# spiraldb/fastlanes

Measured on AMD Instinct MI355X. Metric: billion integers/sec decoded (u32 width-7) + achieved HBM GB/s vs peak, 1-8 GPU, higher is better.
Workload: dtype u32

## Files before the change

fastlanes_amd/csrc/fl_pair.hip:

```cpp
#include "../../include/fastlanes_amd.h"
#include "../../include/fastlanes_amd_internal.h"
#include "fl_host.hpp"
#include "fl_stream.hpp"

#include <algorithm>
#include <atomic>
#include <cmath>
#include <memory>
#include <mutex>
#include <new>
#include <vector>

namespace {

using namespace fl;

int probe_classes(char* base, size_t n, size_t piece, int* classes, hipStream_t s)
{
    constexpr unsigned PROBE_WIDTH = 20;
    const size_t probe_blocks = std::min<size_t>(2000000, piece / (128 * PROBE_WIDTH));
    const size_t mask_off = piece - std::min<size_t>(piece / 2, (size_t)1 << 30);
    for (size_t g = 0; g < n; ++g) classes[g] = -1;
    if (n == 0 || probe_blocks == 0) return FL_OK;
    int rc = FL_OK;
    auto probe_ms = [&](size_t gi, size_t gm, float& ms) {
        const uint32_t* src = reinterpret_cast<const uint32_t*>(base + gi * piece);
        uint32_t* mask = reinterpret_cast<uint32_t*>(base + gm * piece + mask_off);
        return median_ms(s, 1, 3, [&] {
            const int saved = fl::window_override_this_thread();
            fl::window_override_this_thread() = fl::WINDOW_WHOLE;
            const int r = fl_u32_unpack_compare(PROBE_WIDTH, src, FL_CMP_LT, 1u << (PROBE_WIDTH - 1), probe_blocks, mask, s);
            fl::window_override_this_thread() = saved;
            return r;
        }, &ms);
    };
    float threshold = 0.f;
    std::vector<float> ms(n);
    for (int c = 0; c < 3 && rc == FL_OK; ++c) {
        size_t rep = 0;
        while (rep < n && classes[rep] != -1) ++rep;
        if (rep == n) break;
        classes[rep] = c;
        rc = fl_fill_random(base + rep * piece, probe_blocks * 128 * PROBE_WIDTH, 17 + rep, s);
        float slowest = 0.f, fastest = 1e30f;
        size_t others = 0;
        for (size_t g = 0; g < n && rc == FL_OK; ++g) {
            if (classes[g] != -1) continue;
            rc = probe_ms(rep, g, ms[g]);
            slowest = std::max(slowest, ms[g]);
            fastest = std::min(fastest, ms[g]);
            ++others;
        }
        if (rc != FL_OK || others == 0) break;
        if (threshold == 0.f) {
            if (slowest - fastest <= 0.05f * slowest) break;
            threshold = 0.5f * (slowest + fastest);
        }
        for (size_t g = 0; g < n; ++g)
            if (classes[g] == -1 && ms[g] > threshold) classes[g] = c;
    }
    return rc;
}

constexpr size_t PAIR_ALIGN = 256, PAIR_ZONE = (size_t)64 << 30, PAIR_MIB = (size_t)1 << 20, PAIR_GIB = (size_t)1 << 30;
constexpr size_t PAIR_INTERLEAVED_MIN = 8 * PAIR_GIB;
inline size_t pair_pad(size_t b) { return (b + PAIR_ALIGN - 1) & ~(PAIR_ALIGN - 1); }


std::mutex g_live_mutex;
std::vector<std::pair<uintptr_t, uintptr_t>> g_live;
std::atomic<int> g_live_count{0};
void live_pair_add(const char* va, size_t bytes)
{
    const uintptr_t lo = reinterpret_cast<uintptr_t>(va);
    std::lock_guard<std::mutex> lock(g_live_mutex);
    g_live.emplace_back(lo, lo + bytes);
    g_live_count.store((int)g_live.size(), std::memory_order_relaxed);
}
void live_pair_remove(const char* va)
{
    const uintptr_t lo = reinterpret_cast<uintptr_t>(va);
    std::lock_guard<std::mutex> lock(g_live_mutex);
    g_live.erase(std::remove_if(g_live.begin(), g_live.end(), [&](const auto& r) { return r.first == lo; }), g_live.end());
    g_live_count.store((int)g_live.size(), std::memory_order_relaxed);
}

constexpr int CACHE_DEVICES = 16;
std::vector<hipMemGenericAllocationHandle_t> g_chunk_cache[CACHE_DEVICES];
size_t g_chunk_cache_limit = 0;
std::atomic_flag g_chunk_cache_lock = ATOMIC_FLAG_INIT;
void recycle_chunk(hipMemGenericAllocationHandle_t h, int dev)
{
    bool kept = false;
    if (dev >= 0 && dev < CACHE_DEVICES) {
        while (g_chunk_cache_lock.test_and_set(std::memory_order_acquire)) {}
        if (g_chunk_cache[dev].size() < g_chunk_cache_limit) { g_chunk_cache[dev].push_back(h); kept = true; }
        g_chunk_cache_lock.clear(std::memory_order_release);
    }
    if (!kept) (void)hipMemRelease(h);
}
bool cached_chunk(int dev, hipMemGenericAllocationHandle_t& h)
{
    bool got = false;
    if (dev >= 0 && dev < CACHE_DEVICES) {
        while (g_chunk_cache_lock.test_and_set(std::memory_order_acquire)) {}
        if (!g_chunk_cache[dev].empty()) { h = g_chunk_cache[dev].back(); g_chunk_cache[dev].pop_back(); got = true; }
        g_chunk_cache_lock.clear(std::memory_order_release);
    }
    return got;
}

struct ColumnPair {
    void* bufs[3] = {nullptr, nullptr, nullptr};
    void *in = nullptr, *aux = nullptr, *out = nullptr;
    std::vector<hipMemGenericAllocationHandle_t> chunks;
    char* va = nullptr;
    size_t va_bytes = 0, chunk_bytes = 0, n_mapped = 0;
    int dev = -1;
    char class_map[96] = {0};
    ColumnPair() = default;
    ColumnPair(const ColumnPair&) = delete;
    ColumnPair& operator=(const ColumnPair&) = delete;
    ~ColumnPair()
    {
        for (void* b : bufs)
            if (b) (void)hipFree(b);
        if (n_mapped) {
            int cur = -1;
            const bool switched = hipGetDevice(&cur) == hipSuccess && cur != dev && hipSetDevice(dev) == hipSuccess;
            (void)hipDeviceSynchronize();
            if (switched) (void)hipSetDevice(cur);
        }
        for (size_t i = 0; i < n_mapped; ++i) (void)hipMemUnmap(va + i * chunk_bytes, chunk_bytes);
        for (auto h : chunks) recycle_chunk(h, dev);
        if (va) { live_pair_remove(va); (void)hipMemAddressFree(va, va_bytes); }
    }
};

std::atomic<uintptr_t> g_va_next{(uintptr_t)0x100000000000ull};
constexpr uintptr_t VA_ARENA_END = (uintptr_t)0x700000000000ull;
std::atomic_flag g_va_lock = ATOMIC_FLAG_INIT;
std::vector<std::pair<uintptr_t, uintptr_t>> g_va_used;

hipError_t reserve_fresh_range(size_t bytes, char** out)
{
    std::vector<void*> rejected;
    hipError_t e = hipErrorOutOfMemory;
    *out = nullptr;
    for (int attempt = 0; attempt < 6 && !*out; ++attempt) {
        const uintptr_t span = ((bytes + PAIR_GIB - 1) & ~(PAIR_GIB - 1)) + PAIR_GIB;
        const uintptr_t hint = g_va_next.fetch_add(span, std::memory_order_relaxed);
        if (hint + span > VA_ARENA_END) { e = hipErrorOutOfMemory; break; }
        void* p = nullptr;
        e = hipMemAddressReserve(&p, bytes, 2 * PAIR_MIB, reinterpret_cast<void*>(hint), 0);
        if (e != hipSuccess) { (void)hipGetLastError(); continue; }
        const uintptr_t lo = reinterpret_cast<uintptr_t>(p), hi = lo + bytes;
        while (g_va_lock.test_and_set(std::memory_order_acquire)) {}
        bool used = false;
        for (const auto& r : g_va_used) used = used || (lo < r.second && r.first < hi);
        if (!used) g_va_used.emplace_back(lo, hi);
        g_va_lock.clear(std::memory_order_release);
        if (used) { rejected.push_back(p); e = hipErrorOutOfMemory; }
        else *out = static_cast<char*>(p);
    }
    for (void* p : rejected) (void)hipMemAddressFree(p, bytes);
    return *out ? hipSuccess : e;
}

void choose_chunks(const std::vector<int>& cls, size_t n_in, size_t n_out, int out_classes, std::vector<int>& order, size_t* kept_out = nullptr)
{
    if (kept_out) *kept_out = 0;
    const size_t n = cls.size();
    order.clear();
    if (out_classes != 2) out_classes = 3;
    std::vector<int> by[4];
    for (size_t g = 0; g < n; ++g) by[cls[g] < 0 || cls[g] > 2 ? 3 : cls[g]].push_back((int)g);
    if (n_out == 0 || n_in + n_out > n) {
        for (size_t g = 0; g < n_in + n_out && g < n; ++g) order.push_back((int)g);
        return;
    }
    constexpr int TS = 64;
    std::vector<unsigned> pos((size_t)TS * 8);
    for (int t = 0; t < TS; ++t)
        for (int x = 0; x < 8; ++x) {
            const double p = (x + (t + 0.5) / TS) * (double)n_out / 8.0;
            pos[(size_t)t * 8 + x] = (unsigned)std::min<double>((double)n_out - 1, p);
        }
    struct Plan { std::vector<int> label; double cost; size_t kept; };
    auto plan = [&](int c) {
        Plan P;
        size_t avail[4] = {by[0].size(), by[1].size(), by[2].size(), by[3].size()};
        avail[c] -= n_in;
        static const double own_class_fee = [] { const char* e = getenv("FL_INTERNAL_OWN_CLASS_FEE"); return e ? atof(e) : 600.0; }();
        double fee[4] = {0, 0, 0, own_class_fee + 50.0};
        bool in_rotation[3], plentiful = true;
        for (int k = 0; k < 3; ++k) {
            in_rotation[k] = out_classes == 3 || k != c;
            if (in_rotation[k] && avail[k] * (size_t)out_classes < n_out + (size_t)out_classes - 1) plentiful = false;
        }
        for (int k = 0; k < 3; ++k) fee[k] = in_rotation[k] ? 0.0 : plentiful ? own_class_fee : 0.5 * own_class_fee;
        const int S[3] = {(c + 1) % 3, (c + 2) % 3, c};
        P.label.assign(n_out, 0);
        for (size_t j = 0; j < n_out; ++j) {
            const double at = (j + 0.5) * 8.0 / (double)n_out;
            const size_t x = (size_t)at, k = (size_t)((at - (double)x) * (double)n_out / 8.0);
            P.label[j] = S[(x + k) % (size_t)out_classes];
        }
        auto cost_of = [&](const std::vector<int>& lab) {
            double cost = 0.0;
            size_t used[4] = {0, 0, 0, 0};
            for (int k : lab) { ++used[k]; cost += fee[k] / (double)n_out; }
            for (int k = 0; k < 4; ++k) if (used[k] > avail[k]) cost += 10000.0 * (double)(used[k] - avail[k]);
            for (int t = 0; t < TS; ++t) {
                double cnt[4] = {0, 0, 0, 0};
                for (int x = 0; x < 8; ++x) cnt[lab[pos[(size_t)t * 8 + x]]] += 1.0;
                for (int k = 0; k < 4; ++k) cost += cnt[k] * cnt[k] * cnt[k] / TS;
            }
            return cost;
        };
        P.cost = cost_of(P.label);
        for (int sweep = 0; sweep < 12; ++sweep) {
            bool improved = false;
            for (size_t j = 0; j < n_out; ++j) {
                const int was = P.label[j];
                int best = was;
                for (int k = 0; k < 4; ++k) {
                    if (k == was) continue;
                    P.label[j] = k;
                    const double cst = cost_of(P.label);
                    if (cst < P.cost - 1e-9) { P.cost = cst; best = k; }
                }
                P.label[j] = best;
                improved = improved || best != was;
            }
            if (!improved) break;
        }
        size_t used[4] = {0, 0, 0, 0};
        for (int k : P.label) ++used[k];
        double off = 0.0;
        size_t outside = used[3];
        for (int k = 0; k < 3; ++k) {
            if (in_rotation[k]) off += std::max(0.0, std::fabs((double)used[k] - (double)n_out / out_classes) - 1.0);
            else outside += used[k];
        }
        const double kept = (double)n_out - (double)outside - off;
        P.kept = kept > 0.0 ? (size_t)kept : 0;
        for (int k = 0; k < 4; ++k) if (used[k] > avail[k]) P.kept = 0;
        return P;
    };
    int best_c = -1;
    Plan best;
    for (int c = 0; c < 3; ++c) {
        if (by[c].size() < n_in) continue;
        Plan P = plan(c);
        if (best_c < 0 || P.cost < best.cost - 1e-9 || (std::fabs(P.cost - best.cost) <= 1e-9 && by[c].size() > by[best_c].size())) { best = std::move(P); best_c = c; }
    }
    if (best_c < 0) {
        for (size_t g = 0; g < n_in + n_out && g < n; ++g) order.push_back((int)g);
        return;
    }
    if (kept_out) *kept_out = best.kept;
    size_t next[4] = {0, 0, 0, 0};
    for (size_t i = 0; i < n_in; ++i) order.push_back(by[best_c][next[best_c]++]);
    for (size_t j = 0; j < n_out; ++j) {
        int k = best.label[j];
        if (next[k] >= by[k].size()) {
            k = -1;
            for (int q = 0; q < 4; ++q) if (next[q] < by[q].size() && (k < 0 || by[q].size() - next[q] > by[k].size() - next[k])) k = q;
            if (k < 0) break;
        }
        order.push_back(by[k][next[k]++]);
    }
}
}

bool fl::fl_in_constructed_pair(std::initializer_list<const void*> ptrs)
{
    if (g_live_count.load(std::memory_order_relaxed) == 0) return false;
    std::lock_guard<std::mutex> lock(g_live_mutex);
    for (const auto& [lo, hi] : g_live) {
        int inside = 0;
        for (const void* p : ptrs) {
            const uintptr_t a = reinterpret_cast<uintptr_t>(p);
            inside += (a >= lo && a < hi);
        }
        if (inside >= 2) return true;
    }
    return false;
}

namespace {

std::mutex g_construct_mutex;

hipError_t pair_alloc_interleaved(size_t in_bytes, size_t aux_bytes, size_t out_bytes, hipStream_t s, ColumnPair& p, int& rc)
{
    std::lock_guard<std::mutex> one_at_a_time(g_construct_mutex);
    rc = FL_OK;
    int dev = 0, vmm = 0;
    hipError_t e = hipGetDevice(&dev);
    if (e == hipSuccess) e = hipDeviceGetAttribute(&vmm, hipDeviceAttributeVirtualMemoryManagementSupported, dev);
    if (e != hipSuccess) return e;
    if (!vmm) return hipErrorNotSupported;
    const size_t in_span = pair_pad(in_bytes) + pair_pad(aux_bytes), total = in_span + pair_pad(out_bytes);
    const size_t chunk = PAIR_GIB;
    const size_t n_in = std::max<size_t>(1, (in_span + chunk - 1) / chunk), n_out = std::max<size_t>(1, (pair_pad(out_bytes) + chunk - 1) / chunk);
    const int out_classes = pair_pad(out_bytes) >= 3 * in_span ? 2 : 3;
    size_t n_pool = std::max(std::max(std::max(3 * n_in + (out_classes == 3 ? n_out : 0), (3 * n_out + 1) / 2), 2 * (n_in + n_out)), 48 * PAIR_GIB / chunk);
    size_t free_b = 0, total_b = 0;
    if (hipMemGetInfo(&free_b, &total_b) == hipSuccess && free_b > 3 * PAIR_GIB) n_pool = std::min(n_pool, (free_b - 2 * PAIR_GIB) / chunk);
    if (n_pool < n_in + n_out) return hipErrorOutOfMemory;
    hipMemAllocationProp prop{};
    prop.type = hipMemAllocationTypePinned;
    prop.location.type = hipMemLocationTypeDevice;
    prop.location.id = dev;
    hipMemAccessDesc acc{};
    acc.location = prop.location;
    acc.flags = hipMemAccessFlagsProtReadWrite;
    std::vector<hipMemGenericAllocationHandle_t> pool;
    auto drop_pool = [&] { for (auto h : pool) recycle_chunk(h, dev); pool.clear(); };
    p.dev = dev;
    const size_t pool_cap = free_b > 3 * PAIR_GIB ? (free_b - 2 * PAIR_GIB) / chunk : n_pool;
    std::vector<int> cls, order;
    for (int round = 0;; ++round) {
        pool.reserve(n_pool);
        while (pool.size() < n_pool) {
            hipMemGenericAllocationHandle_t h;
            if (!cached_chunk(dev, h) && hipMemCreate(&h, chunk, &prop, 0) != hipSuccess) { (void)hipGetLastError(); break; }
            pool.push_back(h);
        }
        if (pool.size() < n_in + n_out) { drop_pool(); return hipErrorOutOfMemory; }
        cls.assign(pool.size(), -1);
        char* scratch = nullptr;
        e = reserve_fresh_range(pool.size() * chunk, &scratch);
        if (e != hipSuccess) { drop_pool(); return e; }
        size_t mapped = 0;
        for (; mapped < pool.size() && e == hipSuccess; ++mapped) e = hipMemMap(scratch + mapped * chunk, chunk, 0, pool[mapped], 0);
        if (e != hipSuccess) --mapped;
        if (e == hipSuccess) e = hipMemSetAccess(scratch, pool.size() * chunk, &acc, 1);
        if (e == hipSuccess) rc = probe_classes(scratch, pool.size(), chunk, cls.data(), s);
        if (e == hipSuccess && rc == FL_OK) e = hipStreamSynchronize(s);
        for (size_t i = 0; i < mapped; ++i) (void)hipMemUnmap(scratch + i * chunk, chunk);
        (void)hipMemAddressFree(scratch, pool.size() * chunk);
        if (e != hipSuccess || rc != FL_OK) { drop_pool(); return e; }
        size_t kept = 0;
        choose_chunks(cls, n_in, n_out, out_classes, order, &kept);
        const bool complete = order.size() == n_in + n_out;
        const size_t bigger = std::min(std::min(pool_cap, std::max<size_t>(3 * (n_in + n_out), 96)), pool.size() + std::max<size_t>(pool.size() / 2, 8));
        if ((complete && 10 * kept >= 9 * n_out) || round == 3 || pool.size() < n_pool || bigger <= pool.size()) {
            if (!complete) { drop_pool(); return hipErrorOutOfMemory; }
            break;
        }
        n_pool = bigger;
    }
    std::vector<char> keep(pool.size(), 0);
    for (int g : order) keep[g] = 1;
    p.chunk_bytes = chunk;
    p.va_bytes = order.size() * chunk;
    e = reserve_fresh_range(p.va_bytes, &p.va);
    for (size_t i = 0; i < order.size() && e == hipSuccess; ++i) {
        e = hipMemMap(p.va + i * chunk, chunk, 0, pool[order[i]], 0);
        if (e == hipSuccess) p.n_mapped = i + 1;
    }
    if (e == hipSuccess) e = hipMemSetAccess(p.va, p.va_bytes, &acc, 1);
    for (size_t g = 0; g < pool.size(); ++g) {
        if (keep[g]) p.chunks.push_back(pool[g]);
        else recycle_chunk(pool[g], dev);
    }
    pool.clear();
    if (e != hipSuccess) return e;
    for (size_t i = 0; i < order.size() && i + 1 < sizeof p.class_map; ++i) p.class_map[i] = cls[order[i]] < 0 ? '?' : (char)('A' + cls[order[i]]);
    p.in = p.va;
    p.aux = aux_bytes ? p.va + pair_pad(in_bytes) : nullptr;
    p.out = p.va + n_in * chunk;
    live_pair_add(p.va, p.va_bytes);
    return hipSuccess;
}

hipError_t pair_alloc(int layout, size_t in_bytes, size_t aux_bytes, size_t out_bytes, hipStream_t s, ColumnPair& p, int& rc)
{
    rc = FL_OK;
    if (layout == FL_LAYOUT_INTERLEAVED && pair_pad(in_bytes) + pair_pad(aux_bytes) + pair_pad(out_bytes) >= PAIR_INTERLEAVED_MIN)
        return pair_alloc_interleaved(in_bytes, aux_bytes, out_bytes, s, p, rc);
    if (layout == FL_LAYOUT_SEPARATE || layout == FL_LAYOUT_INTERLEAVED) {
        hipError_t e = hipMalloc(&p.bufs[0], in_bytes ? in_bytes : PAIR_ALIGN);
        if (e == hipSuccess && aux_bytes) e = hipMalloc(&p.bufs[1], aux_bytes);
        if (e == hipSuccess) e = hipMalloc(&p.bufs[2], out_bytes ? out_bytes : PAIR_ALIGN);
        if (e != hipSuccess) return e;
        p.in = p.bufs[0]; p.aux = p.bufs[1]; p.out = p.bufs[2];
        return hipSuccess;
    }
    const size_t in_end = pair_pad(in_bytes) + pair_pad(aux_bytes), half = pair_pad(out_bytes) / 2;
    size_t k = 1;
    while (k * PAIR_ZONE < half + in_end) {
        if (++k > 8) return hipErrorOutOfMemory;
    }
    const size_t out_off = (k * PAIR_ZONE - half) & ~(PAIR_ALIGN - 1);
    hipError_t e = hipMalloc(&p.bufs[0], out_off + pair_pad(out_bytes));
    if (e != hipSuccess) return e;
    char* base = static_cast<char*>(p.bufs[0]);
    p.in = base;
    p.aux = aux_bytes ? base + pair_pad(in_bytes) : nullptr;
    p.out = base + out_off;
    return hipSuccess;
}

int pair_probe(const ColumnPair& p, size_t in_bytes, size_t aux_bytes, size_t out_bytes, hipStream_t s, double& gbps)
{
    const size_t big = in_bytes > out_bytes ? in_bytes : out_bytes;
    const size_t n_units = big / 4096;
    gbps = 0.0;
    if (n_units < 1024) return FL_OK;
    auto unit = [&](size_t bytes) { size_t u = bytes / n_units & ~(size_t)15; return u > 4096 ? 4096 : u; };
    BareArgs a{static_cast<const char*>(p.in), static_cast<const char*>(p.aux), static_cast<char*>(p.out), n_units, 0,
               (unsigned)unit(in_bytes), aux_bytes >= n_units * 128 ? 128u : 0u, (unsigned)unit(out_bytes), 63u};
    if (a.out_unit == 0) return FL_OK;
    float ms = 0.f;
    const int rc = median_ms(s, 2, 5, [&] { return hip_status(launch_bare_stream(a, true, a.in_unit > a.out_unit ? 8 : 6, WINDOW_WHOLE, s)); }, &ms);
    if (rc != FL_OK) return rc;
    if (!(ms > 0.f)) return FL_OK;
    gbps = (double)n_units * (a.in_unit + a.aux_unit + a.out_unit) / (ms * 1e6);
    return FL_OK;
}

bool replaces_kept(int cand, double gbps, int kept, double best)
{
    return kept < 0 || gbps > best * (cand == FL_LAYOUT_ZONED ? 1.02 : 1.01);
}
constexpr int PROBE_ORDER[3] = {FL_LAYOUT_INTERLEAVED, FL_LAYOUT_SEPARATE, FL_LAYOUT_ZONED};
}

extern "C" {

int fl_internal_probe_memory_classes(void* slab, size_t slab_bytes, int* classes, void* stream)
{
    const size_t n_granules = slab_bytes / FL_INTERNAL_GRANULE_BYTES;
    if (n_granules == 0) return FL_OK;
    if (!slab || !classes) return FL_ERR_NULL;
    if (misaligned(slab)) return FL_ERR_ALIGN;
    return probe_classes(static_cast<char*>(slab), n_granules, FL_INTERNAL_GRANULE_BYTES, classes, static_cast<hipStream_t>(stream));
}

int fl_column_pair_alloc(size_t in_bytes, size_t aux_bytes, size_t out_bytes, int layout, void* stream, void** in, void** aux, void** out,
                         void** handle, int* layout_kept, uint32_t* probe_gbps)
{
    if (!in || !out || !handle || (aux_bytes && !aux)) return FL_ERR_NULL;
    if (layout < 0 || layout >= FL_LAYOUT_COUNT) return FL_ERR_INDEX;
    FL_DEVICE_TIER(stream);
    hipStream_t s = static_cast<hipStream_t>(stream);
    *in = *out = *handle = nullptr;
    if (aux) *aux = nullptr;
    if (probe_gbps) for (int i = 0; i < FL_LAYOUT_COUNT; ++i) probe_gbps[i] = 0;
    std::unique_ptr<ColumnPair> kept;
    int kept_layout = -1;
    const size_t biggest = in_bytes > out_bytes ? in_bytes : out_bytes;
    if (layout == FL_LAYOUT_PROBE && biggest / 4096 < 1024) layout = FL_LAYOUT_SEPARATE;
    if (layout != FL_LAYOUT_PROBE) {
        kept.reset(new (std::nothrow) ColumnPair);
        if (!kept) return hip_fail(hipErrorOutOfMemory);
        int rc = FL_OK;
        if (hipError_t e = pair_alloc(layout, in_bytes, aux_bytes, out_bytes, s, *kept, rc); e != hipSuccess || rc != FL_OK)
            return rc != FL_OK ? rc : hip_fail(e);
        kept_layout = layout;
    } else {
        double best = -1.0;
        const bool large = pair_pad(in_bytes) + pair_pad(aux_bytes) + pair_pad(out_bytes) >= PAIR_INTERLEAVED_MIN;
        for (int cand : PROBE_ORDER) {
            if (cand == FL_LAYOUT_INTERLEAVED && !large) continue;
            std::unique_ptr<ColumnPair> p(new (std::nothrow) ColumnPair);
            int prc = FL_OK;
            if (!p || pair_alloc(cand, in_bytes, aux_bytes, out_bytes, s, *p, prc) != hipSuccess || prc != FL_OK) { (void)hipGetLastError(); continue; }
            double gbps = 0.0;
            if (const int r = pair_probe(*p, in_bytes, aux_bytes, out_bytes, s, gbps); r != FL_OK) return r;
            if (probe_gbps) probe_gbps[cand] = (uint32_t)(gbps + 0.5);
            if (replaces_kept(cand, gbps, kept_layout, best)) { kept = std::move(p); best = gbps; kept_layout = cand; }
        }
        if (!kept) return hip_fail(hipErrorOutOfMemory);
    }
    *in = kept->in;
    if (aux) *aux = kept->aux;
    *out = kept->out;
    if (layout_kept) *layout_kept = kept_layout;
    *handle = kept.release();
    return FL_OK;
}

int fl_column_pair_free(void* handle)
{
    delete static_cast<ColumnPair*>(handle);
    return FL_OK;
}

size_t fl_internal_pair_chunk_cache(size_t max_chunks)
{
    std::vector<hipMemGenericAllocationHandle_t> drop;
    size_t held = 0;
    while (g_chunk_cache_lock.test_and_set(std::memory_order_acquire)) {}
    g_chunk_cache_limit = max_chunks;
    for (auto& c : g_chunk_cache) {
        while (c.size() > max_chunks) { drop.push_back(c.back()); c.pop_back(); }
        held += c.size();
    }
    g_chunk_cache_lock.clear(std::memory_order_release);
    for (auto h : drop) (void)hipMemRelease(h);
    return held;
}

size_t fl_internal_choose_chunks(const int* classes, size_t n_pool, size_t n_in, size_t n_out, int out_classes, int* order)
{
    if (!classes || !order || n_pool == 0) return 0;
    std::vector<int> cls(classes, classes + n_pool), chosen;
    choose_chunks(cls, n_in, n_out, out_classes, chosen);
    for (size_t i = 0; i < chosen.size(); ++i) order[i] = chosen[i];
    return chosen.size();
}

int fl_internal_choose_layout(const double* gbps)
{
    int kept = -1;
    double best = -1.0;
    for (int cand : PROBE_ORDER)
        if (gbps && gbps[cand] >= 0.0 && replaces_kept(cand, gbps[cand], kept, best)) { kept = cand; best = gbps[cand]; }
    return kept;
}

const char* fl_internal_column_pair_classes(const void* handle)
{
    return handle ? static_cast<const ColumnPair*>(handle)->class_map : "";
}

}
```

include/fastlanes_amd_internal.h:

```cpp
#ifndef FASTLANES_AMD_INTERNAL_H
#define FASTLANES_AMD_INTERNAL_H

#include <stddef.h>
#include <stdint.h>

#ifdef __cplusplus
extern "C" {
#endif

void fl_internal_set_kernel_policy(int policy);
int fl_internal_get_kernel_policy(void);
uint64_t fl_internal_zero_copy_fallbacks(void);

#define FL_INTERNAL_GRANULE_BYTES ((size_t)8 << 30)
int fl_internal_probe_memory_classes(void *slab, size_t slab_bytes, int *classes, void *stream);

const char *fl_internal_column_pair_classes(const void *handle);

size_t fl_internal_pair_chunk_cache(size_t max_chunks);

size_t fl_internal_choose_chunks(const int *classes, size_t n_pool, size_t n_in, size_t n_out, int out_classes, int *order);

int fl_internal_choose_layout(const double *gbps);

int fl_internal_bare_stream(const void *in, size_t in_unit, const void *aux, size_t aux_unit, void *out, size_t out_unit,
                            size_t n_units, int nt_loads, int waves, int window_log2_units, void *stream);
int fl_internal_bare_stream_shape(int op, unsigned type_bits, unsigned width, size_t *in_unit, size_t *aux_unit, size_t *out_unit,
                                  int *nt_loads, int *waves, int *window_log2_units, unsigned *blocks_per_unit);

int fl_internal_selftune_check(int op, unsigned type_bits, unsigned width, const void *in, const void *aux, void *out, size_t n_blocks,
                               void *stream, float *table_ms, float *best_other_ms, int *best_other_policy);

#ifdef __cplusplus
}
#endif
#endif
```

Baseline: 1421.

## Lower interleaved-layout threshold, cache chunk probe classes, round-robin small outputs

The interleaved VMM layout now applies whenever the larger side (input plus aux, or output) reaches about 3.75 GiB, replacing the old 8 GiB total threshold. More workloads therefore get class-balanced chunk placement across memory channels. Recycled chunks now remember their probed memory class, so a pool made entirely of chunks from the same earlier probe skips the re-probe. Outputs of 8 or fewer chunks get a simple round-robin class labelling before refinement. Counters for created, probed and reused chunks are added. The risk is that cached classes go stale, and that smaller sizes now pay the probe and VMM setup cost.

```diff
diff --git a/fastlanes_amd/csrc/fl_pair.hip b/fastlanes_amd/csrc/fl_pair.hip
--- a/fastlanes_amd/csrc/fl_pair.hip
+++ b/fastlanes_amd/csrc/fl_pair.hip
@@ -63,8 +63,12 @@
 }
 
 constexpr size_t PAIR_ALIGN = 256, PAIR_ZONE = (size_t)64 << 30, PAIR_MIB = (size_t)1 << 20, PAIR_GIB = (size_t)1 << 30;
-constexpr size_t PAIR_INTERLEAVED_MIN = 8 * PAIR_GIB;
 inline size_t pair_pad(size_t b) { return (b + PAIR_ALIGN - 1) & ~(PAIR_ALIGN - 1); }
+constexpr size_t PAIR_INTERLEAVED_MIN_SIDE = 15 * PAIR_GIB / 4;
+inline bool pair_is_constructed(size_t in_bytes, size_t aux_bytes, size_t out_bytes)
+{
+    return std::max(pair_pad(in_bytes) + pair_pad(aux_bytes), pair_pad(out_bytes)) >= PAIR_INTERLEAVED_MIN_SIDE;
+}
 
 
 std::mutex g_live_mutex;
@@ -85,26 +89,32 @@
     g_live_count.store((int)g_live.size(), std::memory_order_relaxed);
 }
 
+struct Chunk {
+    hipMemGenericAllocationHandle_t h;
+    int cls = -1;
+    uint64_t probe = 0;
+};
 constexpr int CACHE_DEVICES = 16;
-std::vector<hipMemGenericAllocationHandle_t> g_chunk_cache[CACHE_DEVICES];
+std::vector<Chunk> g_chunk_cache[CACHE_DEVICES];
 size_t g_chunk_cache_limit = 0;
 std::atomic_flag g_chunk_cache_lock = ATOMIC_FLAG_INIT;
-void recycle_chunk(hipMemGenericAllocationHandle_t h, int dev)
+uint64_t g_probe_number = 0;
+void recycle_chunk(const Chunk& c, int dev)
 {
     bool kept = false;
     if (dev >= 0 && dev < CACHE_DEVICES) {
         while (g_chunk_cache_lock.test_and_set(std::memory_order_acquire)) {}
-        if (g_chunk_cache[dev].size() < g_chunk_cache_limit) { g_chunk_cache[dev].push_back(h); kept = true; }
+        if (g_chunk_cache[dev].size() < g_chunk_cache_limit) { g_chunk_cache[dev].push_back(c); kept = true; }
         g_chunk_cache_lock.clear(std::memory_order_release);
     }
-    if (!kept) (void)hipMemRelease(h);
-}
-bool cached_chunk(int dev, hipMemGenericAllocationHandle_t& h)
+    if (!kept) (void)hipMemRelease(c.h);
+}
+bool cached_chunk(int dev, Chunk& c)
 {
     bool got = false;
     if (dev >= 0 && dev < CACHE_DEVICES) {
         while (g_chunk_cache_lock.test_and_set(std::memory_order_acquire)) {}
-        if (!g_chunk_cache[dev].empty()) { h = g_chunk_cache[dev].back(); g_chunk_cache[dev].pop_back(); got = true; }
+        if (!g_chunk_cache[dev].empty()) { c = g_chunk_cache[dev].back(); g_chunk_cache[dev].pop_back(); got = true; }
         g_chunk_cache_lock.clear(std::memory_order_release);
     }
     return got;
@@ -113,7 +123,7 @@
 struct ColumnPair {
     void* bufs[3] = {nullptr, nullptr, nullptr};
     void *in = nullptr, *aux = nullptr, *out = nullptr;
-    std::vector<hipMemGenericAllocationHandle_t> chunks;
+    std::vector<Chunk> chunks;
     char* va = nullptr;
     size_t va_bytes = 0, chunk_bytes = 0, n_mapped = 0;
     int dev = -1;
@@ -206,6 +216,8 @@
             const size_t x = (size_t)at, k = (size_t)((at - (double)x) * (double)n_out / 8.0);
             P.label[j] = S[(x + k) % (size_t)out_classes];
         }
+        if (n_out <= 8)
+            for (size_t j = 0; j < n_out; ++j) P.label[j] = S[j % (size_t)out_classes];
         auto cost_of = [&](const std::vector<int>& lab) {
             double cost = 0.0;
             size_t used[4] = {0, 0, 0, 0};
@@ -317,32 +329,43 @@
     hipMemAccessDesc acc{};
     acc.location = prop.location;
     acc.flags = hipMemAccessFlagsProtReadWrite;
-    std::vector<hipMemGenericAllocationHandle_t> pool;
-    auto drop_pool = [&] { for (auto h : pool) recycle_chunk(h, dev); pool.clear(); };
+    std::vector<Chunk> pool;
+    auto drop_pool = [&] { for (const Chunk& c : pool) recycle_chunk(c, dev); pool.clear(); };
     p.dev = dev;
     const size_t pool_cap = free_b > 3 * PAIR_GIB ? (free_b - 2 * PAIR_GIB) / chunk : n_pool;
     std::vector<int> cls, order;
     for (int round = 0;; ++round) {
         pool.reserve(n_pool);
         while (pool.size() < n_pool) {
-            hipMemGenericAllocationHandle_t h;
-            if (!cached_chunk(dev, h) && hipMemCreate(&h, chunk, &prop, 0) != hipSuccess) { (void)hipGetLastError(); break; }
-            pool.push_back(h);
+            Chunk c;
+            if (cached_chunk(dev, c)) ++fl_internal_pair_chunk_counters[2];
+            else if (hipMemCreate(&c.h, chunk, &prop, 0) == hipSuccess) ++fl_internal_pair_chunk_counters[0];
+            else { (void)hipGetLastError(); break; }
+            pool.push_back(c);
         }
         if (pool.size() < n_in + n_out) { drop_pool(); return hipErrorOutOfMemory; }
         cls.assign(pool.size(), -1);
-        char* scratch = nullptr;
-        e = reserve_fresh_range(pool.size() * chunk, &scratch);
-        if (e != hipSuccess) { drop_pool(); return e; }
-        size_t mapped = 0;
-        for (; mapped < pool.size() && e == hipSuccess; ++mapped) e = hipMemMap(scratch + mapped * chunk, chunk, 0, pool[mapped], 0);
-        if (e != hipSuccess) --mapped;
-        if (e == hipSuccess) e = hipMemSetAccess(scratch, pool.size() * chunk, &acc, 1);
-        if (e == hipSuccess) rc = probe_classes(scratch, pool.size(), chunk, cls.data(), s);
-        if (e == hipSuccess && rc == FL_OK) e = hipStreamSynchronize(s);
-        for (size_t i = 0; i < mapped; ++i) (void)hipMemUnmap(scratch + i * chunk, chunk);
-        (void)hipMemAddressFree(scratch, pool.size() * chunk);
-        if (e != hipSuccess || rc != FL_OK) { drop_pool(); return e; }
+        bool remembered = pool[0].probe != 0;
+        for (const Chunk& c : pool) remembered = remembered && c.probe == pool[0].probe;
+        if (remembered) {
+            for (size_t g = 0; g < pool.size(); ++g) cls[g] = pool[g].cls;
+        } else {
+            char* scratch = nullptr;
+            e = reserve_fresh_range(pool.size() * chunk, &scratch);
+            if (e != hipSuccess) { drop_pool(); return e; }
+            size_t mapped = 0;
+            for (; mapped < pool.size() && e == hipSuccess; ++mapped) e = hipMemMap(scratch + mapped * chunk, chunk, 0, pool[mapped].h, 0);
+            if (e != hipSuccess) --mapped;
+            if (e == hipSuccess) e = hipMemSetAccess(scratch, pool.size() * chunk, &acc, 1);
+            if (e == hipSuccess) rc = probe_classes(scratch, pool.size(), chunk, cls.data(), s);
+            if (e == hipSuccess && rc == FL_OK) e = hipStreamSynchronize(s);
+            for (size_t i = 0; i < mapped; ++i) (void)hipMemUnmap(scratch + i * chunk, chunk);
+            (void)hipMemAddressFree(scratch, pool.size() * chunk);
+            if (e != hipSuccess || rc != FL_OK) { drop_pool(); return e; }
+            fl_internal_pair_chunk_counters[1] += pool.size();
+            ++g_probe_number;
+            for (size_t g = 0; g < pool.size(); ++g) { pool[g].cls = cls[g]; pool[g].probe = g_probe_number; }
+        }
         size_t kept = 0;
         choose_chunks(cls, n_in, n_out, out_classes, order, &kept);
         const bool complete = order.size() == n_in + n_out;
@@ -359,7 +382,7 @@
     p.va_bytes = order.size() * chunk;
     e = reserve_fresh_range(p.va_bytes, &p.va);
     for (size_t i = 0; i < order.size() && e == hipSuccess; ++i) {
-        e = hipMemMap(p.va + i * chunk, chunk, 0, pool[order[i]], 0);
+        e = hipMemMap(p.va + i * chunk, chunk, 0, pool[order[i]].h, 0);
         if (e == hipSuccess) p.n_mapped = i + 1;
     }
     if (e == hipSuccess) e = hipMemSetAccess(p.va, p.va_bytes, &acc, 1);
@@ -380,7 +403,7 @@
 hipError_t pair_alloc(int layout, size_t in_bytes, size_t aux_bytes, size_t out_bytes, hipStream_t s, ColumnPair& p, int& rc)
 {
     rc = FL_OK;
-    if (layout == FL_LAYOUT_INTERLEAVED && pair_pad(in_bytes) + pair_pad(aux_bytes) + pair_pad(out_bytes) >= PAIR_INTERLEAVED_MIN)
+    if (layout == FL_LAYOUT_INTERLEAVED && pair_is_constructed(in_bytes, aux_bytes, out_bytes))
         return pair_alloc_interleaved(in_bytes, aux_bytes, out_bytes, s, p, rc);
     if (layout == FL_LAYOUT_SEPARATE || layout == FL_LAYOUT_INTERLEAVED) {
         hipError_t e = hipMalloc(&p.bufs[0], in_bytes ? in_bytes : PAIR_ALIGN);
@@ -464,9 +487,9 @@
         kept_layout = layout;
     } else {
         double best = -1.0;
-        const bool large = pair_pad(in_bytes) + pair_pad(aux_bytes) + pair_pad(out_bytes) >= PAIR_INTERLEAVED_MIN;
+        const bool constructed = pair_is_constructed(in_bytes, aux_bytes, out_bytes);
         for (int cand : PROBE_ORDER) {
-            if (cand == FL_LAYOUT_INTERLEAVED && !large) continue;
+            if (cand == FL_LAYOUT_INTERLEAVED && !constructed) continue;
             std::unique_ptr<ColumnPair> p(new (std::nothrow) ColumnPair);
             int prc = FL_OK;
             if (!p || pair_alloc(cand, in_bytes, aux_bytes, out_bytes, s, *p, prc) != hipSuccess || prc != FL_OK) { (void)hipGetLastError(); continue; }
@@ -493,7 +516,7 @@
 
 size_t fl_internal_pair_chunk_cache(size_t max_chunks)
 {
-    std::vector<hipMemGenericAllocationHandle_t> drop;
+    std::vector<Chunk> drop;
     size_t held = 0;
     while (g_chunk_cache_lock.test_and_set(std::memory_order_acquire)) {}
     g_chunk_cache_limit = max_chunks;
@@ -502,9 +525,11 @@
         held += c.size();
     }
     g_chunk_cache_lock.clear(std::memory_order_release);
-    for (auto h : drop) (void)hipMemRelease(h);
+    for (const Chunk& c : drop) (void)hipMemRelease(c.h);
     return held;
 }
+
+uint64_t fl_internal_pair_chunk_counters[3] = {0, 0, 0};
 
 size_t fl_internal_choose_chunks(const int* classes, size_t n_pool, size_t n_in, size_t n_out, int out_classes, int* order)
 {
diff --git a/include/fastlanes_amd_internal.h b/include/fastlanes_amd_internal.h
--- a/include/fastlanes_amd_internal.h
+++ b/include/fastlanes_amd_internal.h
@@ -19,6 +19,8 @@
 
 size_t fl_internal_pair_chunk_cache(size_t max_chunks);
 
+extern uint64_t fl_internal_pair_chunk_counters[3];
+
 size_t fl_internal_choose_chunks(const int *classes, size_t n_pool, size_t n_in, size_t n_out, int out_classes, int *order);
 
 int fl_internal_choose_layout(const double *gbps);
```

New measurement: 1421, median of 3. No clear change (+0.0%).
